# harvard-edge/multilingual_kws

Hardware: AMD Instinct MI355X
Metric: clips/sec end-to-end (log-mel + embedding fwd), batch 1024, 1s@16kHz (higher is better)
Workload: dtype f32; 1 GPU; configs[2]: batch=1024/GPU synthetic 1s@16kHz clips -> micro-frontend (int16 fixed-point, fp32 I/O) -> EfficientNet-B0 embedding forward (frozen, fp32 MFMA pointwise conv) -> [1024,1024]; clips_per_gpu=1024, samples_per_clip=16000, weights=synthetic seed 1234, parallelism=clip-sharded x1, build=19cccf80cf25db1a

## Files before the change

multilingual_kws_amd/csrc/mkws_embed.hip:

```cpp
#include "mkws_common.h"
#include "mkws_embed_arch.h"

#include <algorithm>
#include <cmath>
#include <cstdlib>
#include <map>
#include <mutex>
#include <new>
#include <set>
#include <string>
#include <type_traits>
#include <vector>

#pragma clang fp contract(fast)
#include "mkws_embed_dev.h"
#include "mkws_embed_rows.h"

namespace mkws {

__device__ __forceinline__ int opaque_(int v) { asm volatile("" : "+v"(v)); return v; }
__device__ __forceinline__ float apply_act(float v, int act) {
  switch (act) {
    case ACT_SWISH: return swishf_(v);
    case ACT_RELU: return v > 0.0f ? v : 0.0f;
// ... 913 lines not shown
template <int NTWR, int DEPTH, typename WP>
__device__ __forceinline__ void stream_mfma_prefetch(f32x4 (&wq)[DEPTH][NTWR], WP wlane, size_t chunk_stride, int tile0,
                                                     int tstride, int ntiles, int KC) {
  if (KC >= DEPTH) {
#pragma unroll
    for (int d = 0; d < DEPTH; ++d)
#pragma unroll
      for (int q = 0; q < NTWR; ++q) {
        int t = tile0 + tstride * q;
        if (t >= ntiles) t = ntiles - 1;
        wq[d][q] = wload(wlane, (size_t)t * 256 + (size_t)d * chunk_stride);
      }
  }
}

template <int NTW, int DEPTH, int MT, bool PRE, int NTWR, typename WP, typename XL, typename XM>
__device__ __forceinline__ void stream_mfma(f32x4 (&acc)[NTW][MT], f32x4 (&wq)[DEPTH][NTWR], WP wlane, size_t chunk_stride,
                                            int tile0, int tstride, int ntiles, int KC, XL xload, XM xmake) {
  size_t wt[NTW];
#pragma unroll
  for (int q = 0; q < NTW; ++q) {
    int t = tile0 + tstride * q;
    if (t >= ntiles) t = ntiles - 1;
    wt[q] = (size_t)t * 256;
  }
  auto load = [&](int j, f32x4 (&wv)[NTWR]) {
#pragma unroll
    for (int q = 0; q < NTW; ++q) wv[q] = wload(wlane, wt[q] + (size_t)j * chunk_stride);
  };
  constexpr int XB = (DEPTH % 2 == 0) ? 2 : DEPTH;
  decltype(xload(0, 0)) xr[XB][MT];
  if (KC > 0) {
#pragma unroll
// ... 21 lines not shown
  };
  if (KC >= DEPTH) {
    if (!PRE) {
#pragma unroll
      for (int d = 0; d < DEPTH; ++d) load(d, wq[d]);
    }
    int j = 0;
    for (; j + 2 * DEPTH <= KC; j += DEPTH) {
#pragma unroll
      for (int d = 0; d < DEPTH; ++d) {
        compute(d, j + d, wq[d]);
        load(j + DEPTH + d, wq[d]);
        __builtin_amdgcn_sched_barrier(0);
      }
    }
#pragma unroll
    for (int d = 0; d < DEPTH; ++d) {
      compute(d, j + d, wq[d]);
      if (j + DEPTH + d < KC) load(j + DEPTH + d, wq[d]);
      __builtin_amdgcn_sched_barrier(0);
    }
    j += DEPTH;
#pragma unroll
    for (int d = 0; d < DEPTH; ++d)
      if (j + d < KC) compute(d, j + d, wq[d]);
  } else {
#pragma unroll
    for (int d = 0; d < DEPTH; ++d)
      if (d < KC) load(d, wq[d]);
#pragma unroll
    for (int d = 0; d < DEPTH; ++d)
      if (d < KC) compute(d, d, wq[d]);
  }
  if (SPLIT) acc[0][0] += acc_odd;
}

template <int KS, int S, int KCT, int HT, int WT, int CEXP, int CC, int G, int SEG>
struct MidGeom {
  static constexpr int HW = HT * WT;
  static constexpr int HoT = (S == 1) ? HT : (HT + 1) / 2, WoT = (S == 1) ? WT : (WT + 1) / 2;
  static constexpr int HoWo = HoT * WoT;
  static constexpr int PT = (S == 1) ? KS / 2 : KS / 2 - (1 - HT % 2), PLF = (S == 1) ? KS / 2 : KS / 2 - (1 - WT % 2);
  static constexpr int NSEG = WoT / SEG;
  static constexpr int NC = (SEG - 1) * S + KS;
// ... 1032 lines not shown

constexpr int kChainMax = 6;
struct ChainArgs {
  const BlockArgs* tab;
  int i0, n;
  unsigned kinds;
  const float* X; float* Y;
  int B;
  int ldsU, ldsE;
  int se4;
#ifdef MKWS_FRONT_TIMING
  unsigned long long* dbg_t;
#endif
};

__device__ __forceinline__ int sgpr_(int v) { return __builtin_amdgcn_readfirstlane(v); }
template <typename T>
__device__ __forceinline__ T* sgpr_(T* p) {
  const unsigned long long v = reinterpret_cast<unsigned long long>(p);
  const unsigned lo = (unsigned)__builtin_amdgcn_readfirstlane((int)(unsigned)v), hi = (unsigned)__builtin_amdgcn_readfirstlane((int)(unsigned)(v >> 32));
  typedef __attribute__((address_space(1))) T* gptr_t;
  return (T*)reinterpret_cast<gptr_t>(((unsigned long long)hi << 32) | lo);
}
__device__ __forceinline__ BlockArgs sgpr_block_args(const BlockArgs& t) {
  BlockArgs a;
  a.X = nullptr; a.Cin = sgpr_(t.Cin);
  a.WpE = sgpr_(t.WpE); a.scE = sgpr_(t.scE); a.shE = sgpr_(t.shE); a.KCe = sgpr_(t.KCe); a.NTe = sgpr_(t.NTe);
  a.Wd = sgpr_(t.Wd); a.scD = sgpr_(t.scD); a.shD = sgpr_(t.shD);
  a.WrP = sgpr_(t.WrP); a.br = sgpr_(t.br); a.NTR = sgpr_(t.NTR); a.We2P = sgpr_(t.We2P); a.be = sgpr_(t.be);
  a.WpP = sgpr_(t.WpP); a.scP = sgpr_(t.scP); a.shP = sgpr_(t.shP); a.NTp = sgpr_(t.NTp);
  a.Y = nullptr; a.Cout = sgpr_(t.Cout); a.residual = sgpr_(t.residual);
  a.dbg_dw = nullptr; a.dbg_gate = nullptr;
  a.B = 0; a.Cexp = sgpr_(t.Cexp); a.se = sgpr_(t.se);
  a.WrQ = sgpr_(t.WrQ); a.We2Q = sgpr_(t.We2Q); a.seT0 = sgpr_(t.seT0); a.seNQ = sgpr_(t.seNQ);
#ifdef MKWS_FRONT_TIMING
  a.dbg_t = nullptr;
#endif
  return a;
}

template <int KS, int S, int MT, int NWAVES>
__device__ __forceinline__ void chain_block(const BlockArgs& a, const BlockArgs* nxp, bool has_next, float* s_blk, int ldsU, int ldsE, bool first,
                                            f32x4 (&carry)[MT], unsigned long long* dbg_t) {
  constexpr int NTHR = NWAVES * 64;
  const BlockArgs* nx = has_next ? nxp : nullptr;
  constexpr int HT = 4, WT = 3, HW = HT * WT;
  constexpr int G = MT * 16 / HW;
  constexpr int HoT = (S == 1) ? HT : 2, WoT = (S == 1) ? WT : 2;
  constexpr int HoWo = HoT * WoT;
  constexpr int MTO = (G * HoWo + 15) / 16;
  constexpr int PT = (S == 1) ? KS / 2 : KS / 2 - (1 - HT % 2), PLF = (S == 1) ? KS / 2 : KS / 2 - (1 - WT % 2);
  constexpr int LDR = 52;
  constexpr int NTWA = (MT >= 3) ? 1 : 2;
  const int Cexp = a.Cexp, LDE = Cexp + 4;
  const int KCx = Cexp / 16;
  float* s_X = s_blk;
  float* s_S = s_blk;
  float* s_G = s_S + G * Cexp;
  float* s_P = s_G;
  float* s_E = s_blk + ldsU;
  float* s_scE = s_E + ldsE;
  float* s_shE = s_scE + Cexp;
  float* s_R = s_scE;
  float* s_be = s_R + 16 * LDR;
  const int tid = opaque_((int)threadIdx.x), lane = tid & 63;
  const int wave = __builtin_amdgcn_readfirstlane(tid >> 6);
  const int g = lane >> 4, c = lane & 15;
  const unsigned loff = (unsigned)(g * 64 + c * 4);
  const int b0 = blockIdx.x * G;
  const int gvalid = (a.B - b0 < G) ? (a.B - b0) : G;
  const int rows_in = gvalid * HW, rows_out = gvalid * HoWo;
  const size_t row0_in = (size_t)b0 * HW, row0_out = (size_t)b0 * HoWo;

#ifdef MKWS_FRONT_TIMING
  if (dbg_t && threadIdx.x == 0) dbg_t[0] = wall_clock64();
#endif
  const int a_groups = (a.NTe + NTWA - 1) / NTWA;
  const int a_runs = (a_groups > wave) ? (a_groups - wave + NWAVES - 1) / NWAVES : 0;
  auto a_tile_of = [&](int r) { return (wave + NWAVES * r) * NTWA; };
  {
    f32x4 wqa[4][NTWA];
    stream_mfma_runs_prefetch<NTWA, 4>(wqa, WBuf(a.WpE, loff), (size_t)a.NTe * 256, a.NTe, a_runs, a.KCe, a_tile_of);
    auto xload = [&](int j, int m) { return *reinterpret_cast<const f32x4*>(s_X + ((size_t)(j * MT + m) * 64 + lane) * 4); };
    auto xmake = [](const f32x4& v) { return v; };
    auto epi = [&](int t0, const f32x4 (&acc)[NTWA][MT]) {
#pragma unroll
      for (int q = 0; q < NTWA; ++q) {
        const int n = (t0 + q) * 16 + 4 * g;
        if (t0 + q < a.NTe) {
          const f32x4 sc = *reinterpret_cast<const f32x4*>(s_scE + n), sh = *reinterpret_cast<const f32x4*>(s_shE + n);
#pragma unroll
          for (int m = 0; m < MT; ++m) {
            f32x4 y = acc[q][m] * sc + sh;
            y = swish4_(y);
            if (m * 16 + c >= rows_in) y = (f32x4){0.f, 0.f, 0.f, 0.f};
            *reinterpret_cast<f32x4*>(s_E + (size_t)(m * 16 + c) * LDE + n) = y;
          }
// ... 1 lines not shown
      }
    };
    stream_mfma_runs<NTWA, 4, MT, true>(wqa, WBuf(a.WpE, loff), (size_t)a.NTe * 256, a.NTe, a_runs, a.KCe, a_tile_of, xload, xmake, epi);
  }
  __syncthreads();

#ifdef MKWS_FRONT_TIMING
  if (dbg_t && threadIdx.x == 0) dbg_t[1] = wall_clock64();
#endif
  for (int i = tid; i < Cexp; i += NTHR) s_be[i] = a.be[i];
  const int c1_per = (KCx + NWAVES - 1) / NWAVES;
  const int c1_j0 = wave * c1_per;
  const int c1_kc = (c1_j0 + c1_per <= KCx) ? c1_per : (KCx > c1_j0 ? KCx - c1_j0 : 0);
  const WBuf c1_w(a.WrP + (size_t)c1_j0 * a.NTR * 256, loff);
  f32x4 wq1[3][3];
  constexpr bool kWq1Early = (KS == 3);
  const bool se4 = a.WrQ != nullptr;
  f32x4 wq4[kSe4MaxTQ];
  if (kWq1Early) {
    if (se4) se4_request_c1(wq4, a.WrQ, wave, lane);
    else stream_mfma_prefetch<3, 3>(wq1, c1_w, (size_t)a.NTR * 256, 0, 1, a.NTR, c1_kc);
  }
  {
    const int Q = Cexp / 4;
    for (int task = tid; task < G * Q; task += NTHR) {
      const int gi = MKWS_DW_CLIP_MINOR ? task % G : task / Q, q4 = (MKWS_DW_CLIP_MINOR ? task / G : task - gi * Q) * 4;
      float* Eg = s_E + (size_t)gi * HW * LDE + q4;
      constexpr int PRE = (KS == 5) ? (MT >= 3 ? 3 : 2) : KS;
      auto tap_used = [](int i, int jx) {
        bool used = false;
        for (int oh = 0; oh < HoT; ++oh)
// ... 58 lines not shown

#ifdef MKWS_FRONT_TIMING
  if (dbg_t && threadIdx.x == 0) dbg_t[2] = wall_clock64();
#endif
  constexpr int NCST = 3;
  float nsc[NCST], nsh[NCST];
  const int nxCexp = nx ? sgpr_(nx->Cexp) : 0;
  if (nx) {
    const float* nscE = sgpr_(nx->scE); const float* nshE = sgpr_(nx->shE);
#pragma unroll
    for (int k = 0; k < NCST; ++k) {
      const int i = tid + k * NTHR;
      if (i < nxCexp) { nsc[k] = nscE[i]; nsh[k] = nshE[i]; }
    }
  }
  constexpr int NTW2 = 3;
  const int c2_groups = (KCx + NTW2 - 1) / NTW2;
  const int c2_runs = (c2_groups > wave) ? (c2_groups - wave + NWAVES - 1) / NWAVES : 0;
  auto c2_tile_of = [&](int r) { return (wave + NWAVES * r) * NTW2; };
  f32x4 wq2[3][NTW2];
  f32x4 wg4[kSe4MaxGroups][kSe4MaxNQ];
  if (se4) {
    se4_c1<G, NWAVES>(wq4, a.seT0, Cexp, s_S, s_P, wave, lane);
    se4_request_c2<NWAVES>(wg4, a.We2Q, Cexp, wave, lane);
    const float br4 = (tid < 32 * G && (tid & 31) < a.se) ? a.br[tid & 31] : 0.0f;
    __syncthreads();
    se4_fold<G, NWAVES, LDR>(s_P, s_R, a.se, br4, tid);
    __syncthreads();
  } else {
    {
// ... 108 lines not shown
    auto xmake = [](const f32x4& v) { return v; };
    auto finish = [&](f32x4 y, int t, int m, int slot, const f32x4& sc, const f32x4& sh) {
      const int n = t * 16 + 4 * g, r = m * 16 + c;
      y = y * sc + sh;
      if (a.residual) {
        if (first) { if (r < rows_out) y += *reinterpret_cast<const f32x4*>(a.X + (row0_in + r) * a.Cin + n); }
        else y += carry[slot];
      }
      if (!nx && r < rows_out) *reinterpret_cast<f32x4*>(a.Y + (row0_out + r) * a.Cout + n) = y;
      if constexpr (S == 1) {
        if (r >= rows_out) y = (f32x4){0.f, 0.f, 0.f, 0.f};
        carry[slot] = y;
        if (nx) *reinterpret_cast<f32x4*>(s_X + ((size_t)(t * MT + m) * 64 + lane) * 4) = y;
      }
    };
    auto run = [&](auto ntw_tag) {
      constexpr int NTW = decltype(ntw_tag)::value;
      f32x4 acc[NTW][MTO];
#pragma unroll
      for (int q = 0; q < NTW; ++q)
#pragma unroll
        for (int m = 0; m < MTO; ++m) acc[q][m] = (f32x4){0.f, 0.f, 0.f, 0.f};
      stream_mfma<NTW, 4, MTO, true>(acc, wqd, d_w, cstride, wave, NWAVES, a.NTp, KCx, xload, xmake);
#pragma unroll
      for (int q = 0; q < NTW; ++q) {
        const int t = wave + NWAVES * q;
        if (t < a.NTp) {
          const int n = t * 16 + 4 * g;
          const f32x4 sc = *reinterpret_cast<const f32x4*>(a.scP + n), sh = *reinterpret_cast<const f32x4*>(a.shP + n);
#pragma unroll
          for (int m = 0; m < MTO; ++m) finish(acc[q][m], t, m, (NTW == 1) ? m : 0, sc, sh);
        }
      }
    };
    if (d_row >= 0) {
      const float* er = erow[0];
#pragma unroll
      for (int m = 1; m < MTO; ++m) er = (d_row == m) ? erow[m] : er;
      auto xload1 = [&](int j, int) { return *reinterpret_cast<const f32x4*>(er + 16 * j); };
      f32x4 acc1[1][1] = {{{0.f, 0.f, 0.f, 0.f}}};
      stream_mfma<1, 4, 1, true>(acc1, wqd, d_w, cstride, a.NTp - 1, NWAVES, a.NTp, KCx, xload1, xmake);
      const int n = (a.NTp - 1) * 16 + 4 * g;
      finish(acc1[0][0], a.NTp - 1, d_row, 0, *reinterpret_cast<const f32x4*>(a.scP + n), *reinterpret_cast<const f32x4*>(a.shP + n));
    } else if (d_ntw == 1) run(std::integral_constant<int, 1>{});
    else if (d_ntw == 2) run(std::integral_constant<int, 2>{});
    else if (d_ntw >= 3) run(std::integral_constant<int, 3>{});
  }
#ifdef MKWS_FRONT_TIMING
  __syncthreads();
  if (dbg_t && threadIdx.x == 0) dbg_t[6] = wall_clock64();
#else
  if (nx) __syncthreads();
#endif
}

template <int MT, int NWAVES>
__global__ __launch_bounds__(NWAVES * 64) void mbconv_chain_kernel(ChainArgs ca) {
  extern __shared__ __attribute__((aligned(16))) float s_blk[];
  constexpr int NTHR = NWAVES * 64;
  constexpr int HW = 12, G = MT * 16 / HW;
  const BlockArgs* __restrict__ tab = ca.tab + ca.i0;
// ... 13 lines not shown
    const int rows_in = gvalid * HW;
    const size_t row0_in = (size_t)b0 * HW;
    float* s_X = s_blk;
    float* s_scE = s_blk + ca.ldsU + ca.ldsE;
    for (int jm = wave; jm < KCe * MT; jm += NWAVES) {
      const int j = jm / MT, m = jm - j * MT;
      const int r = m * 16 + c;
      f32x4 v = {0.f, 0.f, 0.f, 0.f};
      if (r < rows_in && 16 * j + 4 * g < Cin) v = *reinterpret_cast<const f32x4*>(ca.X + (row0_in + r) * Cin + 16 * j + 4 * g);
      *reinterpret_cast<f32x4*>(s_X + ((size_t)jm * 64 + lane) * 4) = v;
    }
    const float* scE = sgpr_(tab[0].scE); const float* shE = sgpr_(tab[0].shE);
    for (int i = tid; i < Cexp; i += NTHR) { s_scE[i] = scE[i]; s_scE[Cexp + i] = shE[i]; }
    __syncthreads();
  }
  for (int i = 0; i < ca.n; ++i) {
    BlockArgs a = sgpr_block_args(tab[i]);
    const bool last = (i + 1 == ca.n);
    if (!ca.se4) a.WrQ = nullptr;
    a.X = ca.X; a.Y = ca.Y; a.B = ca.B;
    const BlockArgs* nxp = last ? tab + i : tab + i + 1;
    const unsigned kind = (ca.kinds >> (2 * i)) & 3u;
#ifdef MKWS_FRONT_TIMING
    unsigned long long* dt = ca.dbg_t ? ca.dbg_t + ((size_t)blockIdx.x * kChainMax + i) * 8 : nullptr;
    if (dt && threadIdx.x == 0) dt[7] = wall_clock64();
#else
    unsigned long long* dt = nullptr;
#endif
    if (kind == 0) chain_block<3, 1, MT, NWAVES>(a, nxp, !last, s_blk, ca.ldsU, ca.ldsE, i == 0, carry, dt);
    else if (kind == 1) chain_block<5, 1, MT, NWAVES>(a, nxp, !last, s_blk, ca.ldsU, ca.ldsE, i == 0, carry, dt);
    else chain_block<5, 2, MT, NWAVES>(a, nxp, !last, s_blk, ca.ldsU, ca.ldsE, i == 0, carry, dt);
  }
}

#ifdef MKWS_PAIR_NT_STORES
#define MKWS_XSTORE(ptr, val) __builtin_nontemporal_store((val), (ptr))
#else
#define MKWS_XSTORE(ptr, val) (*(ptr) = (val))
#endif

struct PairArgs {
  BlockArgs b;
  float* xc1;
  float* xd;
  int* flags;
  int* err_dev;
// ... 367 lines not shown
struct PairChainArgs {
  const BlockArgs* tab;
  int i0, n;
  unsigned kinds;
  const float* X; float* Y;
  int B;
  int ldsU, ldsE, ldsZ;
  float* xc1;
  float* xd;
  int* flags;
  int* err_dev; int* err_host; int fault;
  const float* top_Wp; const float* top_sc; const float* top_sh; int top_KC, top_NT;
  float* gap;
};
static constexpr int kPairXdAll = 20;

template <int KS, int MT, int NWAVES>
__device__ __forceinline__ void pair_chain_block(const BlockArgs& a, const BlockArgs* nxp, bool has_next, bool first, int blk, const PairChainArgs& pa,
                                                 float* s_blk, int h, int pair, int xcc_expect, unsigned xcc, f32x4 (&carry)[2][MT]) {
  constexpr int NTHR = NWAVES * 64;
  constexpr int HT = 2, WT = 2, HW = 4, G = 4 * MT;
  constexpr int PT = KS / 2, PLF = KS / 2;
  constexpr int LDR = 52;
  constexpr int RDA = 4, NTWA = 3;
  const BlockArgs* nx = has_next ? nxp : nullptr;
  const int b0 = pair * G;
  const int Cexp = a.Cexp, CH = Cexp / 2, LDE = CH + 4;
  const int KH = CH / 16;
  const int KCx = Cexp / 16;
  float* s_X = s_blk;
  float* s_S = s_blk;
  float* s_G = s_S + G * CH;
  float* s_P = s_G;
  float* s_E = s_blk + pa.ldsU;
// ... 5 lines not shown
  const int tid = opaque_((int)threadIdx.x), lane = tid & 63;
  const int wave = __builtin_amdgcn_readfirstlane(tid >> 6);
  const int g = lane >> 4, c = lane & 15;
  const int gvalid = (a.B - b0 < G) ? (a.B - b0) : G;
  const int rows = gvalid * HW;
  const size_t row0 = (size_t)b0 * HW;
  const int chan0 = h * CH;
  const unsigned loff = (unsigned)(g * 64 + c * 4);
  int* fl = pa.flags + ((size_t)pair * kPairChainMax + blk) * 4;

  const int a_groups = (KH + NTWA - 1) / NTWA;
  const int a_nruns = (a_groups > wave) ? (a_groups - wave + NWAVES - 1) / NWAVES : 0;
  auto a_tile_of = [&](int r) { return (wave + NWAVES * r) * NTWA; };
  {
    const WBuf a_w(a.WpE + (size_t)(h * KH) * 256, loff);
    f32x4 wqa[RDA][NTWA];
    stream_mfma_runs_prefetch<NTWA, RDA>(wqa, a_w, (size_t)a.NTe * 256, KH, a_nruns, a.KCe, a_tile_of);
    auto xload = [&](int j, int m) { return *reinterpret_cast<const f32x4*>(s_X + ((size_t)(j * MT + m) * 64 + lane) * 4); };
    auto xmake = [](const f32x4& v) { return v; };
    auto epi = [&](int t0, const f32x4 (&acc)[NTWA][MT]) {
#pragma unroll
      for (int q = 0; q < NTWA; ++q) {
        const int n = (t0 + q) * 16 + 4 * g;
        if (t0 + q < KH) {
          const f32x4 sc = *reinterpret_cast<const f32x4*>(s_scE + n), sh = *reinterpret_cast<const f32x4*>(s_shE + n);
#pragma unroll
          for (int m = 0; m < MT; ++m) {
            f32x4 y = acc[q][m] * sc + sh;
            y = swish4_(y);
            if (m * 16 + c >= rows) y = (f32x4){0.f, 0.f, 0.f, 0.f};
            *reinterpret_cast<f32x4*>(s_E + (size_t)(m * 16 + c) * LDE + n) = y;
          }
// ... 193 lines not shown
      if constexpr (NTW > 0) {
        stream_mfma<NTW, 4, MT, true>(acc, wqd, d_w, cstride, wave, NWAVES, a.NTp, KH, xload, xmake);
        if (sends) {
#pragma unroll
          for (int q = 0; q < NTW; ++q) {
            const int t = wave + NWAVES * q;
            if (t < a.NTp) {
#pragma unroll
              for (int m = 0; m < MT; ++m) MKWS_XSTORE(reinterpret_cast<f32x4*>(xd_mine + ((size_t)(t * 2 + m) * 64 + lane) * 4), acc[q][m]);
            }
          }
        }
      }
      asm volatile("s_waitcnt vmcnt(0)" ::: "memory");
      __syncthreads();
      if (tid == 0 && *s_bad == 0) {
        const int got = pair_signal_wait(fl + 2 + h, fl + 2 + (h ^ 1), 1);
        if (got != 1) { *s_bad = 1; pair_report(pa.err_dev, pa.err_host, kPairErrTimeout); }
      }
      __syncthreads();
      if constexpr (NTW > 0) {
        if (finishes) {
          const bool bad = *s_bad != 0;
#pragma unroll
          for (int q = 0; q < NTW; ++q) {
            const int t = wave + NWAVES * q;
            const int n = t * 16 + 4 * g;
            if (t < a.NTp) {
              const f32x4 sc = *reinterpret_cast<const f32x4*>(a.scP + n), sh = *reinterpret_cast<const f32x4*>(a.shP + n);
#pragma unroll
// ... 12 lines not shown
                if (nx) *reinterpret_cast<f32x4*>(s_X + ((size_t)(t * MT + m) * 64 + lane) * 4) = y;
              }
            }
          }
        }
      }
    };
    if (d_ntw == 0) run(std::integral_constant<int, 0>{});
    else if (d_ntw == 1) run(std::integral_constant<int, 1>{});
    else if (d_ntw == 2) run(std::integral_constant<int, 2>{});
    else run(std::integral_constant<int, 3>{});
  }
  if (nx) __syncthreads();
}

template <int MT, int NWAVES>
__device__ __forceinline__ void pair_top_phase(const PairChainArgs& pa, float* s_blk, int h, int pair) {
  constexpr int G = 4 * MT, NTW = 5;
  const int tid = opaque_((int)threadIdx.x), lane = tid & 63;
  const int wave = __builtin_amdgcn_readfirstlane(tid >> 6);
  const int g = lane >> 4, c = lane & 15;
  const unsigned loff = (unsigned)(g * 64 + c * 4);
  const int b0 = pair * G;
  const int NTh = pa.top_NT / 2;
  const float* s_X = s_blk;
  const WBuf w(pa.top_Wp, loff);
  f32x4 wq[4][NTW];
  f32x4 acc[NTW][MT];
#pragma unroll
  for (int q = 0; q < NTW; ++q)
#pragma unroll
    for (int m = 0; m < MT; ++m) acc[q][m] = (f32x4){0.f, 0.f, 0.f, 0.f};
  auto xload = [&](int j, int m) { return *reinterpret_cast<const f32x4*>(s_X + ((size_t)(j * MT + m) * 64 + lane) * 4); };
  auto xmake = [](const f32x4& v) { return v; };
  stream_mfma<NTW, 4, MT, false>(acc, wq, w, (size_t)pa.top_NT * 256, h * NTh + wave, NWAVES, (h + 1) * NTh, pa.top_KC, xload, xmake);
#pragma unroll
  for (int q = 0; q < NTW; ++q) {
    const int i = wave + NWAVES * q;
    const int n = (h * NTh + i) * 16 + 4 * g;
    const bool tok = i < NTh;
    const f32x4 sc = *reinterpret_cast<const f32x4*>(pa.top_sc + (tok ? n : 0)), sh = *reinterpret_cast<const f32x4*>(pa.top_sh + (tok ? n : 0));
#pragma unroll
    for (int m = 0; m < MT; ++m) {
      f32x4 y = acc[q][m] * sc + sh;
      y = swish4_(y);
      {
#pragma clang fp contract(off)
        y.x += __shfl_xor(y.x, 1); y.y += __shfl_xor(y.y, 1); y.z += __shfl_xor(y.z, 1); y.w += __shfl_xor(y.w, 1);
        y.x += __shfl_xor(y.x, 2); y.y += __shfl_xor(y.y, 2); y.z += __shfl_xor(y.z, 2); y.w += __shfl_xor(y.w, 2);
      }
// ... 33 lines not shown
    const int rows = gvalid * HW;
    const size_t row0 = (size_t)b0 * HW;
    float* s_X = s_blk;
    float* s_scE = s_blk + pa.ldsU + pa.ldsE;
    for (int jm = wave; jm < KCe * MT; jm += NWAVES) {
      const int j = jm / MT, m = jm - j * MT;
      const int r = m * 16 + c;
      f32x4 v = {0.f, 0.f, 0.f, 0.f};
      if (r < rows && 16 * j + 4 * g < Cin) v = *reinterpret_cast<const f32x4*>(pa.X + (row0 + r) * Cin + 16 * j + 4 * g);
      *reinterpret_cast<f32x4*>(s_X + ((size_t)jm * 64 + lane) * 4) = v;
    }
    const float* scE = sgpr_(tab[0].scE) + h * CH; const float* shE = sgpr_(tab[0].shE) + h * CH;
    for (int i = tid; i < CH; i += NTHR) { s_scE[i] = scE[i]; s_scE[CH + i] = shE[i]; }
    __syncthreads();
  }
  for (int i = 0; i < pa.n; ++i) {
    BlockArgs a = sgpr_block_args(tab[i]);
    const bool last = (i + 1 == pa.n);
    a.X = pa.X; a.Y = pa.Y; a.B = pa.B;
    const BlockArgs* nxp = last ? tab + i : tab + i + 1;
    const bool hands_on = !last || pa.top_Wp != nullptr;
    if (((pa.kinds >> i) & 1u) == 0) pair_chain_block<5, MT, NWAVES>(a, nxp, hands_on, i == 0, i, pa, s_blk, h, pair, xcc_expect, xcc, carry);
    else pair_chain_block<3, MT, NWAVES>(a, nxp, hands_on, i == 0, i, pa, s_blk, h, pair, xcc_expect, xcc, carry);
  }
  if (pa.top_Wp != nullptr) pair_top_phase<MT, NWAVES>(pa, s_blk, h, pair);
}

constexpr int kClusterPMax = 14, kClXc1 = 256, kClMaxTiles = 20, kClusterChMax = 192, kClFlagRow = 16;
constexpr int kClusterLdsFloats = 12 * 256 + 16 * (kClusterChMax + 4) + 4 * kClusterChMax + 4 * 52 + 2 * kClusterChMax + 48 * (kClusterChMax + 4) + 48 * kClusterChMax +
                                  27 * kClusterChMax;
struct ClusterArgs {
  BlockArgs b;
  const float* Wr;
  const float* We;
  float* xc1;
  float* xd;
  int* flags;
  int* err_dev; int* err_host; int fault;
  int P;
};
// ... 605 lines not shown
  float *gap = nullptr, *d0 = nullptr, *d1 = nullptr;
  float* se_part = nullptr;
  float* splitk_ws = nullptr; size_t splitk_floats = 0;
  const float *stem_w = nullptr, *stem_scale = nullptr, *stem_shift = nullptr;
  float norm_mean = 0.f, norm_std = 1.f;
  bool fuse_front = true;
  int fuse_gap = 1;
  int fuse_stem = 1;
  int fuse_back = 1;
  int fuse_mid = 1;
  int fuse_gemv = 1;
  int fuse_se4 = 1;
  int fuse_walk = 1;
  int fuse_rows = 0;
  int fuse_block = 2;
  int fuse_chain = 1;
  mkws::BlockArgs* d_chain_tab = nullptr;
  int fuse_top = 1;
  int fuse_pair = 1;
  float* pair_xc1 = nullptr; float* pair_xd = nullptr; int* pair_flags = nullptr;
  int* pair_err_dev = nullptr;
  int* pair_err_host = nullptr;
  size_t pair_flag_count = 0;
  int* pair_chain_flags = nullptr;
  int pair_fault = 0;
  int pair_degraded = 0;
  int fuse_cluster = 0;
  float* cl_xc1 = nullptr; float* cl_xd = nullptr; int* cl_flags = nullptr; size_t cl_flag_count = 0;
  int fuse_cluster_chain = 0;
  int pair_mt = 2;
// ... 397 lines not shown
  if (!em->d_chain_tab) return fail(MKWS_ERR_UNSUPPORTED, "chain: no block table");
  ca.tab = em->d_chain_tab; ca.i0 = i0; ca.n = n; ca.kinds = 0; ca.ldsU = ca.ldsE = 0;
  ca.X = X; ca.Y = Y; ca.B = B; ca.se4 = em->fuse_se4;
  int ldsZ = 0;
  std::string names;
  for (int k = 0; k < n; ++k) {
    const BlockPlan& b = em->blocks[i0 + k];
    const int ks = b.spec.kernel, st = b.spec.stride;
    if (ks == 3 && st != 1) return fail(MKWS_ERR_UNSUPPORTED, "chain: 3x3 stride-2 block");
    ca.kinds |= (unsigned)((ks == 3 && st == 1) ? 0 : (ks == 5 && st == 1) ? 1 : 2) << (2 * k);
    const int MT = block_row_tiles(b, mt43), G = MT * 16 / (b.H * b.W);
    const BlockLds L = block_lds(b.expand.KC, b.ce, MT, G, kBlockWaves);
    ca.ldsU = std::max(ca.ldsU, L.U); ca.ldsE = std::max(ca.ldsE, L.E); ldsZ = std::max(ldsZ, L.Z);
    names += (k ? "," : "") + std::string(b.spec.name);
  }
  const size_t lds = ((size_t)ca.ldsU + ca.ldsE + ldsZ) * sizeof(float);
  if (lds > 160 * 1024) return fail(MKWS_ERR_UNSUPPORTED, "chain: LDS carve %zu bytes", lds);
  const int G = mt43 * 16 / 12;
  const dim3 grid((B + G - 1) / G);
  ProfScope ps("chain:" + names, std::string("mbconv_chain_kernel<") + std::to_string(mt43) + "," + std::to_string(kBlockWaves) + ">");
  void (*k)(ChainArgs);
  if (mt43 == 3) k = &mbconv_chain_kernel<3, kBlockWaves>;
  else if (mt43 == 2) k = &mbconv_chain_kernel<2, kBlockWaves>;
  else k = &mbconv_chain_kernel<1, kBlockWaves>;
  timing_arm(ca, grid.x);
  if (int rc = launch_big_lds(k, 160 * 1024, grid, dim3(kBlockWaves * 64), lds, s, ca)) return rc;
  timing_report_chain(s, em->blocks + i0, n, names, grid.x, ca);
  return MKWS_OK;
}

// ... 75 lines not shown
  for (int k = 0; k < n; ++k) {
    const BlockPlan& b = em->blocks[i0 + k];
    if (b.spec.kernel == 3) pa.kinds |= 1u << k;
    const PairLds L = pair_lds(b.expand.KC, b.ce / 2, mt);
    pa.ldsU = std::max(pa.ldsU, L.U); pa.ldsE = std::max(pa.ldsE, L.E); pa.ldsZ = std::max(pa.ldsZ, L.Z);
    names += (k ? "," : "") + std::string(b.spec.name);
  }
  pa.top_Wp = nullptr; pa.top_sc = pa.top_sh = nullptr; pa.top_KC = pa.top_NT = 0; pa.gap = nullptr;
  if (with_top) {
    const GemmLayer& T = em->top;
    if (T.NTtot != 2 * 5 * kBlockWaves || T.KC < 4 || T.KC != em->blocks[i1].project.NTtot) return fail(MKWS_ERR_UNSUPPORTED, "pair chain: top conv shape");
    pa.top_Wp = T.Wp; pa.top_sc = T.scale; pa.top_sh = T.shift; pa.top_KC = T.KC; pa.top_NT = T.NTtot; pa.gap = em->gap;
    pa.ldsU = std::max(pa.ldsU, T.KC * mt * 256);
    names += ",top";
  }
  const size_t lds = ((size_t)pa.ldsU + pa.ldsE + pa.ldsZ) * sizeof(float);
  if (lds > 160 * 1024) return fail(MKWS_ERR_UNSUPPORTED, "pair chain: LDS carve %zu bytes", lds);
  const dim3 grid(2 * pair_count(B, mt));
  ProfScope ps("chain:" + names, std::string("mbconv_pair_chain_kernel<") + std::to_string(mt) + "," + std::to_string(kBlockWaves) + ">");
  void (*k)(PairChainArgs) = (mt == 2) ? &mbconv_pair_chain_kernel<2, kBlockWaves> : &mbconv_pair_chain_kernel<1, kBlockWaves>;
  return launch_big_lds(k, 160 * 1024, grid, dim3(kBlockWaves * 64), lds, s, pa);
}

constexpr int kClusterMaxBatch = 32;
static int cluster_count(int B, int clips_per_cluster) { return (((B + clips_per_cluster - 1) / clips_per_cluster) + 7) / 8 * 8; }
static int cluster_members(int ce) {
  for (int P = kClusterPMax; P >= 2; --P)
    if (ce % (16 * P) == 0 && ce / P >= 48 && ce / P <= kClusterChMax) return P;
  return 0;
}
// ... 640 lines not shown
  int (*get)(const mkws_embed*);
};
void plan_tiles(mkws_embed* em) { em->pair_mt = pair_row_tiles(em->plan_batch); em->block_mt43 = block43_row_tiles(em->plan_batch); }
const EmbedOption kEmbedOptions[] = {
    {"fuse_front", nullptr, [](mkws_embed* em, int v) { em->fuse_front = v != 0; return (int)MKWS_OK; }, [](const mkws_embed* em) { return em->fuse_front ? 1 : 0; }},
    {"fuse_block", &mkws_embed::fuse_block, nullptr, nullptr},
    {"fuse_mid", &mkws_embed::fuse_mid, nullptr, nullptr},
    {"fuse_rows", &mkws_embed::fuse_rows, nullptr, nullptr},
    {"fuse_walk", &mkws_embed::fuse_walk, nullptr, nullptr},
    {"fuse_se4", nullptr, [](mkws_embed* em, int v) { em->fuse_se4 = v ? 1 : 0; return (int)MKWS_OK; }, [](const mkws_embed* em) { return em->fuse_se4; }},
    {"fuse_gemv", &mkws_embed::fuse_gemv, nullptr, nullptr},
    {"fuse_back", &mkws_embed::fuse_back, nullptr, nullptr},
    {"fuse_pair", &mkws_embed::fuse_pair, nullptr, nullptr},
    {"fuse_chain", &mkws_embed::fuse_chain, nullptr, nullptr},
    {"fuse_top", &mkws_embed::fuse_top, nullptr, nullptr},
    {"fuse_cluster", nullptr,
     [](mkws_embed* em, int v) {
       if (v && !em->cl_flags) return fail(MKWS_ERR_UNSUPPORTED, "fuse_cluster needs a handle of at most 64 clips (max_batch = %d)", em->max_batch);
       em->fuse_cluster = v; return (int)MKWS_OK;
     },
     [](const mkws_embed* em) { return em->fuse_cluster; }},
    {"fuse_cluster_chain", nullptr,
     [](mkws_embed* em, int v) {
       if (v && (em->max_batch != 1 || !em->cl_flags)) return fail(MKWS_ERR_UNSUPPORTED, "fuse_cluster_chain is the plan of one-clip handles (max_batch = %d)", em->max_batch);
       em->fuse_cluster_chain = v; return (int)MKWS_OK;
     },
     [](const mkws_embed* em) { return em->fuse_cluster_chain; }},
    {"fuse_stem", &mkws_embed::fuse_stem, nullptr, nullptr},
    {"fuse_gap", &mkws_embed::fuse_gap, nullptr, nullptr},
    {"big_tiles", nullptr,
// ... 109 lines not shown
```

Baseline: 1.091 million clips/s.

## Prefetch next block's expand weights during project GEMM in fused chain kernels

Adds a specialised sequential path for the known 6-block chain and 4-block pair chain. The blocks are unrolled at compile time, and the first expand-weight chunks for the next block (or the top conv) are requested into a register ring while the current block's project conv finishes its MFMA stream. It also hoists the project scale and shift loads ahead of the stream. The aim is to hide the global-memory latency at each block boundary, at the cost of more register pressure and more code size.

```diff
diff --git a/multilingual_kws_amd/csrc/mkws_embed.hip b/multilingual_kws_amd/csrc/mkws_embed.hip
--- a/multilingual_kws_amd/csrc/mkws_embed.hip
+++ b/multilingual_kws_amd/csrc/mkws_embed.hip
@@ -951,9 +951,10 @@
   }
 }
 
-template <int NTW, int DEPTH, int MT, bool PRE, int NTWR, typename WP, typename XL, typename XM>
+struct NoRequest { __device__ __forceinline__ void operator()() const {} };
+template <int NTW, int DEPTH, int MT, bool PRE, int NTWR, typename WP, typename XL, typename XM, typename AHEAD = NoRequest>
 __device__ __forceinline__ void stream_mfma(f32x4 (&acc)[NTW][MT], f32x4 (&wq)[DEPTH][NTWR], WP wlane, size_t chunk_stride,
-                                            int tile0, int tstride, int ntiles, int KC, XL xload, XM xmake) {
+                                            int tile0, int tstride, int ntiles, int KC, XL xload, XM xmake, AHEAD ahead = AHEAD()) {
   size_t wt[NTW];
 #pragma unroll
   for (int q = 0; q < NTW; ++q) {
@@ -1005,6 +1006,7 @@
         __builtin_amdgcn_sched_barrier(0);
       }
     }
+    ahead();
 #pragma unroll
     for (int d = 0; d < DEPTH; ++d) {
       compute(d, j + d, wq[d]);
@@ -1019,6 +1021,7 @@
 #pragma unroll
     for (int d = 0; d < DEPTH; ++d)
       if (d < KC) load(d, wq[d]);
+    ahead();
 #pragma unroll
     for (int d = 0; d < DEPTH; ++d)
       if (d < KC) compute(d, d, wq[d]);
@@ -2081,6 +2084,10 @@
 #endif
 };
 
+static constexpr unsigned kChainSeqBit = 1u << 31;
+static constexpr int kChainSeqN = 6;
+static constexpr unsigned kChainSeqKinds = kChainSeqBit | (1u << 4) | (1u << 6) | (1u << 8) | (2u << 10);
+
 __device__ __forceinline__ int sgpr_(int v) { return __builtin_amdgcn_readfirstlane(v); }
 template <typename T>
 __device__ __forceinline__ T* sgpr_(T* p) {
@@ -2106,9 +2113,10 @@
   return a;
 }
 
-template <int KS, int S, int MT, int NWAVES>
+template <int MT> constexpr int kChainNtwa = (MT >= 3) ? 1 : 2;
+template <int KS, int S, int MT, int NWAVES, bool SEQ = false>
 __device__ __forceinline__ void chain_block(const BlockArgs& a, const BlockArgs* nxp, bool has_next, float* s_blk, int ldsU, int ldsE, bool first,
-                                            f32x4 (&carry)[MT], unsigned long long* dbg_t) {
+                                            f32x4 (&carry)[MT], unsigned long long* dbg_t, f32x4 (&seq_ring)[4][kChainNtwa<MT>]) {
   constexpr int NTHR = NWAVES * 64;
   const BlockArgs* nx = has_next ? nxp : nullptr;
   constexpr int HT = 4, WT = 3, HW = HT * WT;
@@ -2118,7 +2126,7 @@
   constexpr int MTO = (G * HoWo + 15) / 16;
   constexpr int PT = (S == 1) ? KS / 2 : KS / 2 - (1 - HT % 2), PLF = (S == 1) ? KS / 2 : KS / 2 - (1 - WT % 2);
   constexpr int LDR = 52;
-  constexpr int NTWA = (MT >= 3) ? 1 : 2;
+  constexpr int NTWA = kChainNtwa<MT>;
   const int Cexp = a.Cexp, LDE = Cexp + 4;
   const int KCx = Cexp / 16;
   float* s_X = s_blk;
@@ -2146,8 +2154,9 @@
   const int a_runs = (a_groups > wave) ? (a_groups - wave + NWAVES - 1) / NWAVES : 0;
   auto a_tile_of = [&](int r) { return (wave + NWAVES * r) * NTWA; };
   {
-    f32x4 wqa[4][NTWA];
-    stream_mfma_runs_prefetch<NTWA, 4>(wqa, WBuf(a.WpE, loff), (size_t)a.NTe * 256, a.NTe, a_runs, a.KCe, a_tile_of);
+    f32x4 wqa_own[4][NTWA];
+    f32x4 (&wqa)[4][NTWA] = SEQ ? seq_ring : wqa_own;
+    if (!SEQ || first) stream_mfma_runs_prefetch<NTWA, 4>(wqa, WBuf(a.WpE, loff), (size_t)a.NTe * 256, a.NTe, a_runs, a.KCe, a_tile_of);
     auto xload = [&](int j, int m) { return *reinterpret_cast<const f32x4*>(s_X + ((size_t)(j * MT + m) * 64 + lane) * 4); };
     auto xmake = [](const f32x4& v) { return v; };
     auto epi = [&](int t0, const f32x4 (&acc)[NTWA][MT]) {
@@ -2179,7 +2188,7 @@
   const int c1_kc = (c1_j0 + c1_per <= KCx) ? c1_per : (KCx > c1_j0 ? KCx - c1_j0 : 0);
   const WBuf c1_w(a.WrP + (size_t)c1_j0 * a.NTR * 256, loff);
   f32x4 wq1[3][3];
-  constexpr bool kWq1Early = (KS == 3);
+  constexpr bool kWq1Early = (KS == 3) && !SEQ;
   const bool se4 = a.WrQ != nullptr;
   f32x4 wq4[kSe4MaxTQ];
   if (kWq1Early) {
@@ -2268,6 +2277,8 @@
       if (i < nxCexp) { nsc[k] = nscE[i]; nsh[k] = nshE[i]; }
     }
   }
+  const float* nxWpE = (SEQ && nx) ? sgpr_(nx->WpE) : nullptr;
+  const int nxNTe = (SEQ && nx) ? sgpr_(nx->NTe) : 0, nxKCe = (SEQ && nx) ? sgpr_(nx->KCe) : 0;
   constexpr int NTW2 = 3;
   const int c2_groups = (KCx + NTW2 - 1) / NTW2;
   const int c2_runs = (c2_groups > wave) ? (c2_groups - wave + NWAVES - 1) / NWAVES : 0;
@@ -2406,6 +2417,15 @@
         if (nx) *reinterpret_cast<f32x4*>(s_X + ((size_t)(t * MT + m) * 64 + lane) * 4) = y;
       }
     };
+    auto request_next_ring = [&]() {
+      if constexpr (SEQ) {
+        if (nx) {
+          const int n_groups = (nxNTe + NTWA - 1) / NTWA;
+          const int n_runs = (n_groups > wave) ? (n_groups - wave + NWAVES - 1) / NWAVES : 0;
+          stream_mfma_runs_prefetch<NTWA, 4>(seq_ring, WBuf(nxWpE, loff), (size_t)nxNTe * 256, nxNTe, n_runs, nxKCe, a_tile_of);
+        }
+      }
+    };
     auto run = [&](auto ntw_tag) {
       constexpr int NTW = decltype(ntw_tag)::value;
       f32x4 acc[NTW][MTO];
@@ -2413,13 +2433,21 @@
       for (int q = 0; q < NTW; ++q)
 #pragma unroll
         for (int m = 0; m < MTO; ++m) acc[q][m] = (f32x4){0.f, 0.f, 0.f, 0.f};
-      stream_mfma<NTW, 4, MTO, true>(acc, wqd, d_w, cstride, wave, NWAVES, a.NTp, KCx, xload, xmake);
+      f32x4 scq[NTW], shq[NTW];
+      if constexpr (SEQ) {
+#pragma unroll
+        for (int q = 0; q < NTW; ++q) {
+          const int t = (wave + NWAVES * q < a.NTp) ? wave + NWAVES * q : a.NTp - 1;
+          scq[q] = *reinterpret_cast<const f32x4*>(a.scP + t * 16 + 4 * g); shq[q] = *reinterpret_cast<const f32x4*>(a.shP + t * 16 + 4 * g);
+        }
+      }
+      stream_mfma<NTW, 4, MTO, true>(acc, wqd, d_w, cstride, wave, NWAVES, a.NTp, KCx, xload, xmake, request_next_ring);
 #pragma unroll
       for (int q = 0; q < NTW; ++q) {
         const int t = wave + NWAVES * q;
         if (t < a.NTp) {
           const int n = t * 16 + 4 * g;
-          const f32x4 sc = *reinterpret_cast<const f32x4*>(a.scP + n), sh = *reinterpret_cast<const f32x4*>(a.shP + n);
+          const f32x4 sc = SEQ ? scq[q] : *reinterpret_cast<const f32x4*>(a.scP + n), sh = SEQ ? shq[q] : *reinterpret_cast<const f32x4*>(a.shP + n);
 #pragma unroll
           for (int m = 0; m < MTO; ++m) finish(acc[q][m], t, m, (NTW == 1) ? m : 0, sc, sh);
         }
@@ -2431,12 +2459,16 @@
       for (int m = 1; m < MTO; ++m) er = (d_row == m) ? erow[m] : er;
       auto xload1 = [&](int j, int) { return *reinterpret_cast<const f32x4*>(er + 16 * j); };
       f32x4 acc1[1][1] = {{{0.f, 0.f, 0.f, 0.f}}};
-      stream_mfma<1, 4, 1, true>(acc1, wqd, d_w, cstride, a.NTp - 1, NWAVES, a.NTp, KCx, xload1, xmake);
       const int n = (a.NTp - 1) * 16 + 4 * g;
-      finish(acc1[0][0], a.NTp - 1, d_row, 0, *reinterpret_cast<const f32x4*>(a.scP + n), *reinterpret_cast<const f32x4*>(a.shP + n));
+      f32x4 sc1, sh1;
+      if constexpr (SEQ) { sc1 = *reinterpret_cast<const f32x4*>(a.scP + n); sh1 = *reinterpret_cast<const f32x4*>(a.shP + n); }
+      stream_mfma<1, 4, 1, true>(acc1, wqd, d_w, cstride, a.NTp - 1, NWAVES, a.NTp, KCx, xload1, xmake, request_next_ring);
+      if constexpr (!SEQ) { sc1 = *reinterpret_cast<const f32x4*>(a.scP + n); sh1 = *reinterpret_cast<const f32x4*>(a.shP + n); }
+      finish(acc1[0][0], a.NTp - 1, d_row, 0, sc1, sh1);
     } else if (d_ntw == 1) run(std::integral_constant<int, 1>{});
     else if (d_ntw == 2) run(std::integral_constant<int, 2>{});
     else if (d_ntw >= 3) run(std::integral_constant<int, 3>{});
+    else request_next_ring();
   }
 #ifdef MKWS_FRONT_TIMING
   __syncthreads();
@@ -2480,6 +2512,31 @@
     for (int i = tid; i < Cexp; i += NTHR) { s_scE[i] = scE[i]; s_scE[Cexp + i] = shE[i]; }
     __syncthreads();
   }
+  if (ca.kinds == kChainSeqKinds) {
+    f32x4 ring[4][kChainNtwa<MT>];
+    auto seq_block = [&](auto ks_tag, auto s_tag, auto i_tag) {
+      constexpr int KS = decltype(ks_tag)::value, S = decltype(s_tag)::value, I = decltype(i_tag)::value;
+      constexpr bool last = (I + 1 == kChainSeqN);
+      BlockArgs a = sgpr_block_args(tab[I]);
+      if (!ca.se4) a.WrQ = nullptr;
+      a.X = ca.X; a.Y = ca.Y; a.B = ca.B;
+#ifdef MKWS_FRONT_TIMING
+      unsigned long long* dt = ca.dbg_t ? ca.dbg_t + ((size_t)blockIdx.x * kChainMax + I) * 8 : nullptr;
+      if (dt && threadIdx.x == 0) dt[7] = wall_clock64();
+#else
+      unsigned long long* dt = nullptr;
+#endif
+      chain_block<KS, S, MT, NWAVES, true>(a, last ? tab + I : tab + I + 1, !last, s_blk, ca.ldsU, ca.ldsE, I == 0, carry, dt, ring);
+    };
+    using std::integral_constant;
+    seq_block(integral_constant<int, 3>{}, integral_constant<int, 1>{}, integral_constant<int, 0>{});
+    seq_block(integral_constant<int, 3>{}, integral_constant<int, 1>{}, integral_constant<int, 1>{});
+    seq_block(integral_constant<int, 5>{}, integral_constant<int, 1>{}, integral_constant<int, 2>{});
+    seq_block(integral_constant<int, 5>{}, integral_constant<int, 1>{}, integral_constant<int, 3>{});
+    seq_block(integral_constant<int, 5>{}, integral_constant<int, 1>{}, integral_constant<int, 4>{});
+    seq_block(integral_constant<int, 5>{}, integral_constant<int, 2>{}, integral_constant<int, 5>{});
+    return;
+  }
   for (int i = 0; i < ca.n; ++i) {
     BlockArgs a = sgpr_block_args(tab[i]);
     const bool last = (i + 1 == ca.n);
@@ -2493,9 +2550,10 @@
 #else
     unsigned long long* dt = nullptr;
 #endif
-    if (kind == 0) chain_block<3, 1, MT, NWAVES>(a, nxp, !last, s_blk, ca.ldsU, ca.ldsE, i == 0, carry, dt);
-    else if (kind == 1) chain_block<5, 1, MT, NWAVES>(a, nxp, !last, s_blk, ca.ldsU, ca.ldsE, i == 0, carry, dt);
-    else chain_block<5, 2, MT, NWAVES>(a, nxp, !last, s_blk, ca.ldsU, ca.ldsE, i == 0, carry, dt);
+    f32x4 no_ring[4][kChainNtwa<MT>];
+    if (kind == 0) chain_block<3, 1, MT, NWAVES>(a, nxp, !last, s_blk, ca.ldsU, ca.ldsE, i == 0, carry, dt, no_ring);
+    else if (kind == 1) chain_block<5, 1, MT, NWAVES>(a, nxp, !last, s_blk, ca.ldsU, ca.ldsE, i == 0, carry, dt, no_ring);
+    else chain_block<5, 2, MT, NWAVES>(a, nxp, !last, s_blk, ca.ldsU, ca.ldsE, i == 0, carry, dt, no_ring);
   }
 }
 
@@ -2893,10 +2951,13 @@
   float* gap;
 };
 static constexpr int kPairXdAll = 20;
-
-template <int KS, int MT, int NWAVES>
+static constexpr int kPairSeqN = 4;
+static constexpr unsigned kPairSeqKinds = kChainSeqBit | (1u << 3);
+
+template <int KS, int MT, int NWAVES, bool SEQ = false, typename REQ = NoRequest>
 __device__ __forceinline__ void pair_chain_block(const BlockArgs& a, const BlockArgs* nxp, bool has_next, bool first, int blk, const PairChainArgs& pa,
-                                                 float* s_blk, int h, int pair, int xcc_expect, unsigned xcc, f32x4 (&carry)[2][MT]) {
+                                                 float* s_blk, int h, int pair, int xcc_expect, unsigned xcc, f32x4 (&carry)[2][MT],
+                                                 f32x4 (&seq_ring)[4][3], REQ request_next = REQ()) {
   constexpr int NTHR = NWAVES * 64;
   constexpr int HT = 2, WT = 2, HW = 4, G = 4 * MT;
   constexpr int PT = KS / 2, PLF = KS / 2;
@@ -2932,8 +2993,9 @@
   auto a_tile_of = [&](int r) { return (wave + NWAVES * r) * NTWA; };
   {
     const WBuf a_w(a.WpE + (size_t)(h * KH) * 256, loff);
-    f32x4 wqa[RDA][NTWA];
-    stream_mfma_runs_prefetch<NTWA, RDA>(wqa, a_w, (size_t)a.NTe * 256, KH, a_nruns, a.KCe, a_tile_of);
+    f32x4 wqa_own[RDA][NTWA];
+    f32x4 (&wqa)[RDA][NTWA] = SEQ ? seq_ring : wqa_own;
+    if (!SEQ || first) stream_mfma_runs_prefetch<NTWA, RDA>(wqa, a_w, (size_t)a.NTe * 256, KH, a_nruns, a.KCe, a_tile_of);
     auto xload = [&](int j, int m) { return *reinterpret_cast<const f32x4*>(s_X + ((size_t)(j * MT + m) * 64 + lane) * 4); };
     auto xmake = [](const f32x4& v) { return v; };
     auto epi = [&](int t0, const f32x4 (&acc)[NTWA][MT]) {
@@ -3157,6 +3219,7 @@
       }
       asm volatile("s_waitcnt vmcnt(0)" ::: "memory");
       __syncthreads();
+      if constexpr (SEQ) request_next();
       if (tid == 0 && *s_bad == 0) {
         const int got = pair_signal_wait(fl + 2 + h, fl + 2 + (h ^ 1), 1);
         if (got != 1) { *s_bad = 1; pair_report(pa.err_dev, pa.err_host, kPairErrTimeout); }
@@ -3199,8 +3262,13 @@
   if (nx) __syncthreads();
 }
 
-template <int MT, int NWAVES>
-__device__ __forceinline__ void pair_top_phase(const PairChainArgs& pa, float* s_blk, int h, int pair) {
+template <int NWAVES>
+__device__ __forceinline__ void pair_top_request(f32x4 (&wq)[4][5], const PairChainArgs& pa, int h, int wave, unsigned loff) {
+  const int NTh = pa.top_NT / 2;
+  stream_mfma_prefetch<5, 4>(wq, WBuf(pa.top_Wp, loff), (size_t)pa.top_NT * 256, h * NTh + wave, NWAVES, (h + 1) * NTh, pa.top_KC);
+}
+template <int MT, int NWAVES, bool PRE = false>
+__device__ __forceinline__ void pair_top_phase(const PairChainArgs& pa, float* s_blk, int h, int pair, f32x4 (&wq)[4][5]) {
   constexpr int G = 4 * MT, NTW = 5;
   const int tid = opaque_((int)threadIdx.x), lane = tid & 63;
   const int wave = __builtin_amdgcn_readfirstlane(tid >> 6);
@@ -3210,7 +3278,6 @@
   const int NTh = pa.top_NT / 2;
   const float* s_X = s_blk;
   const WBuf w(pa.top_Wp, loff);
-  f32x4 wq[4][NTW];
   f32x4 acc[NTW][MT];
 #pragma unroll
   for (int q = 0; q < NTW; ++q)
@@ -3218,7 +3285,7 @@
     for (int m = 0; m < MT; ++m) acc[q][m] = (f32x4){0.f, 0.f, 0.f, 0.f};
   auto xload = [&](int j, int m) { return *reinterpret_cast<const f32x4*>(s_X + ((size_t)(j * MT + m) * 64 + lane) * 4); };
   auto xmake = [](const f32x4& v) { return v; };
-  stream_mfma<NTW, 4, MT, false>(acc, wq, w, (size_t)pa.top_NT * 256, h * NTh + wave, NWAVES, (h + 1) * NTh, pa.top_KC, xload, xmake);
+  stream_mfma<NTW, 4, MT, PRE>(acc, wq, w, (size_t)pa.top_NT * 256, h * NTh + wave, NWAVES, (h + 1) * NTh, pa.top_KC, xload, xmake);
 #pragma unroll
   for (int q = 0; q < NTW; ++q) {
     const int i = wave + NWAVES * q;
@@ -3282,16 +3349,49 @@
     for (int i = tid; i < CH; i += NTHR) { s_scE[i] = scE[i]; s_scE[CH + i] = shE[i]; }
     __syncthreads();
   }
+  if (pa.kinds == kPairSeqKinds) {
+    f32x4 ring[4][3];
+    f32x4 top_ring[4][5];
+    const unsigned loff = (unsigned)(g * 64 + c * 4);
+    auto seq_block = [&](auto ks_tag, auto i_tag, auto request_next) {
+      constexpr int KS = decltype(ks_tag)::value, I = decltype(i_tag)::value;
+      constexpr bool last = (I + 1 == kPairSeqN);
+      BlockArgs a = sgpr_block_args(tab[I]);
+      a.X = pa.X; a.Y = pa.Y; a.B = pa.B;
+      pair_chain_block<KS, MT, NWAVES, true>(a, last ? tab + I : tab + I + 1, true, I == 0, I, pa, s_blk, h, pair, xcc_expect, xcc, carry, ring, request_next);
+    };
+    auto ring_of = [&](int I) {
+      const float* W = sgpr_(tab[I].WpE);
+      const int NTe = sgpr_(tab[I].NTe), KCe = sgpr_(tab[I].KCe), KH = sgpr_(tab[I].Cexp) / 32;
+      return [=, &ring]() {
+        const int groups = (KH + 2) / 3;
+        const int nruns = (groups > wave) ? (groups - wave + NWAVES - 1) / NWAVES : 0;
+        stream_mfma_runs_prefetch<3, 4>(ring, WBuf(W + (size_t)(h * KH) * 256, loff), (size_t)NTe * 256, KH, nruns, KCe,
+                                        [=](int r) { return (wave + NWAVES * r) * 3; });
+      };
+    };
+    using std::integral_constant;
+    seq_block(integral_constant<int, 5>{}, integral_constant<int, 0>{}, ring_of(1));
+    seq_block(integral_constant<int, 5>{}, integral_constant<int, 1>{}, ring_of(2));
+    seq_block(integral_constant<int, 5>{}, integral_constant<int, 2>{}, ring_of(3));
+    seq_block(integral_constant<int, 3>{}, integral_constant<int, 3>{}, [&]() { pair_top_request<NWAVES>(top_ring, pa, h, wave, loff); });
+    pair_top_phase<MT, NWAVES, true>(pa, s_blk, h, pair, top_ring);
+    return;
+  }
+  f32x4 no_ring[4][3];
   for (int i = 0; i < pa.n; ++i) {
     BlockArgs a = sgpr_block_args(tab[i]);
     const bool last = (i + 1 == pa.n);
     a.X = pa.X; a.Y = pa.Y; a.B = pa.B;
     const BlockArgs* nxp = last ? tab + i : tab + i + 1;
     const bool hands_on = !last || pa.top_Wp != nullptr;
-    if (((pa.kinds >> i) & 1u) == 0) pair_chain_block<5, MT, NWAVES>(a, nxp, hands_on, i == 0, i, pa, s_blk, h, pair, xcc_expect, xcc, carry);
-    else pair_chain_block<3, MT, NWAVES>(a, nxp, hands_on, i == 0, i, pa, s_blk, h, pair, xcc_expect, xcc, carry);
-  }
-  if (pa.top_Wp != nullptr) pair_top_phase<MT, NWAVES>(pa, s_blk, h, pair);
+    if (((pa.kinds >> i) & 1u) == 0) pair_chain_block<5, MT, NWAVES>(a, nxp, hands_on, i == 0, i, pa, s_blk, h, pair, xcc_expect, xcc, carry, no_ring);
+    else pair_chain_block<3, MT, NWAVES>(a, nxp, hands_on, i == 0, i, pa, s_blk, h, pair, xcc_expect, xcc, carry, no_ring);
+  }
+  if (pa.top_Wp != nullptr) {
+    f32x4 wq[4][5];
+    pair_top_phase<MT, NWAVES>(pa, s_blk, h, pair, wq);
+  }
 }
 
 constexpr int kClusterPMax = 14, kClXc1 = 256, kClMaxTiles = 20, kClusterChMax = 192, kClFlagRow = 16;
@@ -3927,6 +4027,7 @@
   int fuse_walk = 1;
   int fuse_rows = 0;
   int fuse_block = 2;
+  int chain_seq = 1;
   int fuse_chain = 1;
   mkws::BlockArgs* d_chain_tab = nullptr;
   int fuse_top = 1;
@@ -4354,6 +4455,7 @@
     ca.ldsU = std::max(ca.ldsU, L.U); ca.ldsE = std::max(ca.ldsE, L.E); ldsZ = std::max(ldsZ, L.Z);
     names += (k ? "," : "") + std::string(b.spec.name);
   }
+  if (em->chain_seq && n == kChainSeqN && (ca.kinds | kChainSeqBit) == kChainSeqKinds) ca.kinds |= kChainSeqBit;
   const size_t lds = ((size_t)ca.ldsU + ca.ldsE + ldsZ) * sizeof(float);
   if (lds > 160 * 1024) return fail(MKWS_ERR_UNSUPPORTED, "chain: LDS carve %zu bytes", lds);
   const int G = mt43 * 16 / 12;
@@ -4459,6 +4561,7 @@
     pa.ldsU = std::max(pa.ldsU, T.KC * mt * 256);
     names += ",top";
   }
+  if (em->chain_seq && with_top && n == kPairSeqN && (pa.kinds | kChainSeqBit) == kPairSeqKinds) pa.kinds |= kChainSeqBit;
   const size_t lds = ((size_t)pa.ldsU + pa.ldsE + pa.ldsZ) * sizeof(float);
   if (lds > 160 * 1024) return fail(MKWS_ERR_UNSUPPORTED, "pair chain: LDS carve %zu bytes", lds);
   const dim3 grid(2 * pair_count(B, mt));
@@ -5129,6 +5232,7 @@
     {"fuse_pair", &mkws_embed::fuse_pair, nullptr, nullptr},
     {"fuse_chain", &mkws_embed::fuse_chain, nullptr, nullptr},
     {"fuse_top", &mkws_embed::fuse_top, nullptr, nullptr},
+    {"chain_seq", nullptr, [](mkws_embed* em, int v) { em->chain_seq = v ? 1 : 0; return (int)MKWS_OK; }, [](const mkws_embed* em) { return em->chain_seq; }},
     {"fuse_cluster", nullptr,
      [](mkws_embed* em, int v) {
        if (v && !em->cl_flags) return fail(MKWS_ERR_UNSUPPORTED, "fuse_cluster needs a handle of at most 64 clips (max_batch = %d)", em->max_batch);
```

Result: faster. 1.107 million clips/s (median of 6 runs) (+1.5%).
